# martinhoT/Footsies-Gym

Hardware: NVIDIA B200
Metric: env_frames_per_sec (higher is better)
Workload: dtype int32+fp32

## Files before the change

### footsies_gym_b200/csrc/footsies_kernels.cu

```cuda
#include <sched.h>
#include <stdlib.h>
#include <algorithm>

#include "rollout_kernel.h"
#include "step_kernel.cuh"

using namespace fg;
using namespace fgk;

namespace {

thread_local char g_err[512] = "";
int fail(int code, const char *fmt, const char *detail = "") {
    snprintf(g_err, sizeof g_err, fmt, detail);
    return code;
}
#define CUDA_TRY(expr) do { cudaError_t _e = (expr); if (_e != cudaSuccess) \
    return fail(FG_ERR_CUDA, #expr ": %s", cudaGetErrorString(_e)); } while (0)

}

struct fg_handle {
    fg_config cfg;
    fg_buffers buf;
    bool bound;
    Tables *d_tables;
    int sm_count;
    int64_t launches;
    int64_t step_calls;
    uint8_t *d_mask;
    int large_shape_min_envs;
    int pdl_min_envs;
    int host_chunk_envs;
    int host_lead_div;
    uint4 *d_packed;
    float *d_reward_table;
    uint32_t *d_pack_error;
    float h_reward_table[FG_PACKED_REWARD_TABLE_SIZE];
    int reward_table_count;
    float2 *d_position;
    uint8_t *d_obs_u8;
    cudaStream_t s_compute, s_copy;
    cudaEvent_t ev_fork, ev_join;
    std::vector<cudaEvent_t> ev_slice;
};

namespace {

int grid_for(const fg_handle *h, int blocks_per_sm) {
    int want = (h->cfg.num_envs + kThreads - 1) / kThreads;
    int cap = h->sm_count * blocks_per_sm;
    return want < cap ? (want > 0 ? want : 1) : cap;
}

Params make_params(const fg_handle *h, int first = 0, int count = -1) {
    Params p;
    memset(&p, 0, sizeof p);
    const size_t o = (size_t)first;
    p.pl_f1 = (uint4 *)h->buf.state[FG_PLANE_F1] + o; p.pl_f2 = (uint4 *)h->buf.state[FG_PLANE_F2] + o;
    p.pl_env = (uint4 *)h->buf.state[FG_PLANE_ENV] + o; p.pl_rng = (uint4 *)h->buf.state[FG_PLANE_RNG] + o;
    p.stats = (unsigned long long *)h->buf.stats;
    p.act1 = h->buf.actions_p1 ? h->buf.actions_p1 + o : nullptr;
    p.act2 = h->buf.actions_p2 ? h->buf.actions_p2 + o : nullptr;
    p.obs = (float4 *)h->buf.obs + 2 * o; p.reward = h->buf.reward + o; p.terminated = h->buf.terminated + o;
    p.info_frame = h->buf.info_frame + o; p.info_misc = (uint32_t *)h->buf.info_misc + o;
    p.step_mask = h->buf.step_mask ? h->buf.step_mask + o : nullptr;
    p.tables = h->d_tables;
    p.first_env_index = h->cfg.first_env_index + first;
    p.reverse = (int)(h->step_calls & 1);
    p.pdl = (count < 0 ? h->cfg.num_envs - first : count) >= h->pdl_min_envs;
    p.n = count < 0 ? h->cfg.num_envs - first : count; p.frame_skip = h->cfg.frame_skip; p.autoreset = h->cfg.autoreset;
    p.stale_intro = h->cfg.stale_intro_input;
    p.skip_unactionable = h->cfg.skip_unactionable;
    p.large_shape_min_envs = h->large_shape_min_envs;
    return p;
}

template <bool KF>
cudaError_t launch_step_k(const fg_config &c, int sm_count, cudaStream_t s, const Params &p) {
    const bool d = c.dense_reward != 0, m = p.step_mask != nullptr;
    if (c.p1_bot && c.p2_bot) return launch_step_d<KF, true, true>(d, m, sm_count, s, p);
    if (c.p1_bot) return launch_step_d<KF, true, false>(d, m, sm_count, s, p);
    if (c.p2_bot) return launch_step_d<KF, false, true>(d, m, sm_count, s, p);
    return launch_step_d<KF, false, false>(d, m, sm_count, s, p);
}

template <bool B1, bool B2>
cudaError_t launch_reset(int grid, cudaStream_t s, const Params &p) {
    static DeviceOnceFlags configured;
    if (cudaError_t e = configure_once_per_device(configured, [] {
            return cudaFuncSetAttribute(reset_kernel<B1, B2>, cudaFuncAttributeMaxDynamicSharedMemorySize, (int)sizeof(Tables)); }))
        return e;
    reset_kernel<B1, B2><<<grid, kThreads, sizeof(Tables), s>>>(p);
    return cudaSuccess;
}

int check_bound(const fg_handle *h) {
    if (!h) return fail(FG_ERR_INVALID_ARGUMENT, "null handle%s");
    if (!h->bound) return fail(FG_ERR_NOT_BOUND, "fg_bind has not been called%s");
    return FG_OK;
}

struct HostOut {
    float *obs_f32;
    float *position;
    uint8_t *obs_u8;
    float *reward;
    uint8_t *terminated;
    int32_t *info_frame;
    uint8_t *info_misc;
};

__global__ void __launch_bounds__(256) pack_obs_kernel(const float4 *__restrict__ obs, float2 *__restrict__ position,
                                                        uint8_t *__restrict__ obs_u8, int n) {
    const int pairs = n >> 1;
    for (int j = blockIdx.x * blockDim.x + threadIdx.x; j < pairs; j += gridDim.x * blockDim.x) {
        const float4 a0 = obs[4 * (size_t)j], a1 = obs[4 * (size_t)j + 1], b0 = obs[4 * (size_t)j + 2], b1 = obs[4 * (size_t)j + 3];
        reinterpret_cast<float4 *>(position)[j] = make_float4(a1.z, a1.w, b1.z, b1.w);
        const uint32_t A[6] = { (uint32_t)a0.x, (uint32_t)a0.y, (uint32_t)a0.z, (uint32_t)a0.w, (uint32_t)a1.x, (uint32_t)a1.y };
        const uint32_t B[6] = { (uint32_t)b0.x, (uint32_t)b0.y, (uint32_t)b0.z, (uint32_t)b0.w, (uint32_t)b1.x, (uint32_t)b1.y };
        uint32_t *o = reinterpret_cast<uint32_t *>(obs_u8) + 3 * (size_t)j;
        o[0] = A[0] | A[1] << 8 | A[2] << 16 | A[3] << 24;
        o[1] = A[4] | A[5] << 8 | B[0] << 16 | B[1] << 24;
        o[2] = B[2] | B[3] << 8 | B[4] << 16 | B[5] << 24;
    }
    if ((n & 1) && blockIdx.x == 0 && threadIdx.x == 0) {
        const int i = n - 1;
        const float4 a0 = obs[2 * (size_t)i], a1 = obs[2 * (size_t)i + 1];
        position[i] = make_float2(a1.z, a1.w);
        const float v[6] = { a0.x, a0.y, a0.z, a0.w, a1.x, a1.y };
        for (int k = 0; k < 6; k++) obs_u8[6 * (size_t)i + k] = (uint8_t)v[k];
    }
}

__global__ void __launch_bounds__(256) delay_ring_kernel(const float4 *__restrict__ obs, const int32_t *__restrict__ frame,
                                                         const uint32_t *__restrict__ misc, float4 *ring_obs, int32_t *ring_frame,
                                                         uint32_t *ring_misc, float4 *__restrict__ out_obs, int32_t *__restrict__ out_frame,
                                                         uint32_t *__restrict__ out_misc, const uint8_t *__restrict__ step_mask,
                                                         int n, int depth, int pos) {
    const int oldest = (pos + 1) % depth;
    for (int i = blockIdx.x * blockDim.x + threadIdx.x; i < n; i += gridDim.x * blockDim.x) {
        const int32_t f_now = frame[i];
        if ((step_mask && !step_mask[i]) || (f_now != -1 && f_now == ring_frame[(size_t)((pos + depth - 1) % depth) * n + i])) {
            const size_t last = (size_t)(depth - 1) * n + i;
            float4 ca = ring_obs[2 * last], cb = ring_obs[2 * last + 1];
            int32_t cf = ring_frame[last];
            uint32_t cm = ring_misc[last];
            for (int s = 0; s < depth; s++) {
                const size_t k = (size_t)s * n + i;
                const float4 ta = ring_obs[2 * k], tb = ring_obs[2 * k + 1];
                const int32_t tf = ring_frame[k];
                const uint32_t tm = ring_misc[k];
                ring_obs[2 * k] = ca; ring_obs[2 * k + 1] = cb; ring_frame[k] = cf; ring_misc[k] = cm;
                ca = ta; cb = tb; cf = tf; cm = tm;
            }
            continue;
        }
// ... 311 lines not shown
    if (cudaGetDeviceCount(&ndev) != cudaSuccess || device < 0 || device >= ndev) {
        cudaGetLastError();
        fail(FG_ERR_INVALID_ARGUMENT, "fg_host_alloc: no such device%s");
        return nullptr;
    }
    if (cudaSetDevice(device) != cudaSuccess) { fail(FG_ERR_CUDA, "fg_host_alloc: cudaSetDevice failed%s"); return nullptr; }
    cpu_set_t old_set, node_set;
    const int node = gpu_numa_node(device);
    const bool have_old = sched_getaffinity(0, sizeof old_set, &old_set) == 0;
    const bool bound = node >= 0 && have_old && node_cpuset(node, &node_set) && sched_setaffinity(0, sizeof node_set, &node_set) == 0;
    void *p = nullptr;
    cudaError_t e = cudaHostAlloc(&p, bytes ? bytes : 1, cudaHostAllocDefault);
    if (e == cudaSuccess) memset(p, 0, bytes);
    if (bound) sched_setaffinity(0, sizeof old_set, &old_set);
    if (e != cudaSuccess) { cudaGetLastError(); fail(FG_ERR_CUDA, "fg_host_alloc: cudaHostAlloc failed%s"); return nullptr; }
    return p;
}
void fg_host_free(void *p) { if (p) cudaFreeHost(p); }

int32_t fg_packed_reward_table(fg_handle *h, float *table, int32_t *count) {
    if (!h || !table || !count) return fail(FG_ERR_INVALID_ARGUMENT, "null argument%s");
    CUDA_TRY(cudaSetDevice(h->cfg.device));
    if (int rc = packed_init(h)) return rc;
    memcpy(table, h->h_reward_table, sizeof h->h_reward_table);
    *count = h->reward_table_count;
    return FG_OK;
}
int32_t fg_step_host_packed(fg_handle *h, const uint8_t *a1, const uint8_t *a2, fg_packed_result *out, void *stream) {
    return host_step_packed(h, a1, a2, out, (cudaStream_t)stream);
}
int32_t fg_reset_host_packed(fg_handle *h, const uint8_t *mask, fg_packed_result *out, void *stream) {
    return host_reset_packed(h, mask, out, (cudaStream_t)stream);
}

int32_t fg_abi_version(void) { return FG_ABI_VERSION; }
const char *fg_last_error(void) { return g_err; }

int32_t fg_algorithmic_bytes_per_env_step(const fg_config *cfg) {
    if (!cfg) return 0;
    const bool rng = cfg->p1_bot || cfg->p2_bot;
    int state = 2 * 16 * (rng ? 4 : 3);
    int actions = (cfg->p1_bot ? 0 : 1) + (cfg->p2_bot ? 0 : 1);
    return state + actions + 32  + 4  + 1  + 4  + 4 ;
}

int32_t fg_create(const fg_config *cfg, fg_handle **out) {
    if (!cfg || !out) return fail(FG_ERR_INVALID_ARGUMENT, "null argument%s");
    if (cfg->struct_size != (int32_t)sizeof(fg_config)) return fail(FG_ERR_INVALID_ARGUMENT, "fg_config.struct_size mismatch%s");
    if (cfg->num_envs <= 0) return fail(FG_ERR_INVALID_ARGUMENT, "num_envs must be positive%s");
    if (cfg->frame_skip < 1 || cfg->frame_skip > 64) return fail(FG_ERR_INVALID_ARGUMENT, "frame_skip must be in [1, 64]%s");
    if (cfg->skip_unactionable && cfg->p1_bot) return fail(FG_ERR_INVALID_ARGUMENT, "skip_unactionable needs an agent-controlled P1%s");
    int ndev = 0;
    if (cudaGetDeviceCount(&ndev) != cudaSuccess || ndev == 0) {
        cudaGetLastError();
        return fail(FG_ERR_NO_DEVICE, "no CUDA device: this library has no CPU fallback%s");
    }
    if (cfg->device < 0 || cfg->device >= ndev) return fail(FG_ERR_INVALID_ARGUMENT, "device ordinal out of range%s");
    CUDA_TRY(cudaSetDevice(cfg->device));
    fg_handle *h = new (std::nothrow) fg_handle();
    if (!h) return fail(FG_ERR_INVALID_STATE, "out of host memory%s");
    h->cfg = *cfg;
    h->bound = false;
    h->launches = 0;
    h->step_calls = 0;
    h->d_mask = nullptr;
    h->d_position = nullptr; h->d_obs_u8 = nullptr;
    h->d_packed = nullptr; h->d_reward_table = nullptr; h->d_pack_error = nullptr; h->reward_table_count = 0;
    h->s_compute = h->s_copy = nullptr;
    h->ev_fork = h->ev_join = nullptr;
    h->host_chunk_envs = 1024 * 1024;
    h->host_lead_div = 2;
    if (const char *v = getenv("FOOTSIES_B200_HOST_LEAD_DIV")) { const int d = atoi(v); if (d == 1 || d == 2 || d == 4) h->host_lead_div = d; }
    if (const char *v = getenv("FOOTSIES_B200_HOST_CHUNK_ENVS")) {
        const long long c = atoll(v);
        if (c >= 256) h->host_chunk_envs = (int)((c > (1ll << 30) ? (1ll << 30) : c) / 256 * 256);
    }
    h->large_shape_min_envs = kLargeShapeMinEnvs;
    if (const char *v = getenv("FOOTSIES_B200_LARGE_SHAPE_MIN_ENVS")) h->large_shape_min_envs = atoi(v);
    h->pdl_min_envs = (cfg->frame_skip > 1 || cfg->skip_unactionable) ? 262144 : 0;
    if (const char *v = getenv("FOOTSIES_B200_PDL_MIN_ENVS")) h->pdl_min_envs = atoi(v);
    cudaDeviceProp prop;
    CUDA_TRY(cudaGetDeviceProperties(&prop, cfg->device));
    h->sm_count = prop.multiProcessorCount;
    Tables *host = new Tables();
    build_tables(*host);
    cudaError_t e = cudaMalloc(&h->d_tables, sizeof(Tables));
    if (e == cudaSuccess) e = cudaMemcpy(h->d_tables, host, sizeof(Tables), cudaMemcpyHostToDevice);
    delete host;
    if (e != cudaSuccess) { delete h; return fail(FG_ERR_CUDA, "table upload: %s", cudaGetErrorString(e)); }
    *out = h;
    return FG_OK;
}

void fg_destroy(fg_handle *h) {
    if (!h) return;
    cudaSetDevice(h->cfg.device);
    cudaFree(h->d_tables);
    if (h->d_mask) cudaFree(h->d_mask);
    if (h->d_position) cudaFree(h->d_position);
    if (h->d_packed) { cudaFree(h->d_packed); cudaFree(h->d_reward_table); cudaFree(h->d_pack_error); }
    if (h->d_obs_u8) cudaFree(h->d_obs_u8);
    if (h->s_compute) { cudaStreamDestroy(h->s_compute); cudaStreamDestroy(h->s_copy); cudaEventDestroy(h->ev_fork); cudaEventDestroy(h->ev_join); }
    for (cudaEvent_t e : h->ev_slice) cudaEventDestroy(e);
    delete h;
}

int32_t fg_bind(fg_handle *h, const fg_buffers *b) {
    if (!h || !b) return fail(FG_ERR_INVALID_ARGUMENT, "null argument%s");
    if (b->struct_size != (int32_t)sizeof(fg_buffers)) return fail(FG_ERR_INVALID_ARGUMENT, "fg_buffers.struct_size mismatch%s");
    for (int k = 0; k < FG_STATE_PLANES; k++)
        if (!b->state[k] || ((uintptr_t)b->state[k] & 15u)) return fail(FG_ERR_INVALID_ARGUMENT, "state planes must be non-null and 16-byte aligned%s");
    if (!b->stats || !b->obs || !b->reward || !b->terminated || !b->info_frame || !b->info_misc)
        return fail(FG_ERR_INVALID_ARGUMENT, "output buffers must be non-null%s");
    if (((uintptr_t)b->obs & 15u) || ((uintptr_t)b->info_misc & 3u) || ((uintptr_t)b->stats & 7u))
        return fail(FG_ERR_INVALID_ARGUMENT, "obs must be 16-byte, info_misc 4-byte, stats 8-byte aligned%s");
    if (!h->cfg.p1_bot && !b->actions_p1) return fail(FG_ERR_INVALID_ARGUMENT, "actions_p1 is required unless p1_bot%s");
    if (!h->cfg.p2_bot && !b->actions_p2) return fail(FG_ERR_INVALID_ARGUMENT, "actions_p2 is required unless p2_bot%s");
    h->buf = *b;
    h->bound = true;
    return FG_OK;
}

int32_t fg_seed(fg_handle *h, int64_t seed_base, const uint8_t *mask, void *stream) {
    if (int rc = check_bound(h)) return rc;
    CUDA_TRY(cudaSetDevice(h->cfg.device));
    Params p = make_params(h);
    p.mask = mask; p.seed_base = seed_base;
    seed_kernel<<<grid_for(h, 8), kThreads, 0, (cudaStream_t)stream>>>(p);
    h->launches++;
    CUDA_TRY(cudaGetLastError());
    return FG_OK;
}

int32_t fg_reset(fg_handle *h, const uint8_t *mask, void *stream) {
    if (int rc = check_bound(h)) return rc;
    CUDA_TRY(cudaSetDevice(h->cfg.device));
    return reset_on(h, mask, (cudaStream_t)stream);
}

int32_t fg_step(fg_handle *h, void *stream) {
    if (int rc = check_bound(h)) return rc;
    CUDA_TRY(cudaSetDevice(h->cfg.device));
    h->step_calls++;
    return step_range(h, 0, -1, (cudaStream_t)stream);
}

int32_t fg_step_host(fg_handle *h, const uint8_t *a1, const uint8_t *a2, float *obs, float *reward,
                     uint8_t *terminated, int32_t *info_frame, uint8_t *info_misc, void *stream) {
    HostOut o = { obs, nullptr, nullptr, reward, terminated, info_frame, info_misc };
    return host_step(h, a1, a2, o, (cudaStream_t)stream);
}

int32_t fg_step_host_compact(fg_handle *h, const uint8_t *a1, const uint8_t *a2, const fg_host_outputs *out, void *stream) {
    if (!out || out->struct_size != (int32_t)sizeof(fg_host_outputs))
        return fail(FG_ERR_INVALID_ARGUMENT, "fg_host_outputs is null or its struct_size does not match%s");
    HostOut o = { nullptr, out->position, out->obs_u8, out->reward, out->terminated, out->info_frame, out->info_misc };
    return host_step(h, a1, a2, o, (cudaStream_t)stream);
}

int32_t fg_reset_host(fg_handle *h, const uint8_t *mask, float *obs, int32_t *info_frame, uint8_t *info_misc, void *stream) {
    HostOut o = { obs, nullptr, nullptr, nullptr, nullptr, info_frame, info_misc };
    return host_reset(h, mask, o, (cudaStream_t)stream);
}

int32_t fg_reset_host_compact(fg_handle *h, const uint8_t *mask, const fg_host_outputs *out, void *stream) {
    if (!out || out->struct_size != (int32_t)sizeof(fg_host_outputs))
// ... 154 lines not shown
```

### footsies_gym_b200/csrc/frame_logic.cuh

```cuda
#ifndef FOOTSIES_B200_FRAME_LOGIC_CUH
#define FOOTSIES_B200_FRAME_LOGIC_CUH

#include <stdint.h>

#include "state_codec.h"

#if defined(__CUDACC__)
#define FG_DEV __device__ __forceinline__
#define FG_ALIGN16 __align__(16)
namespace fg {
FG_DEV float u2f(uint32_t u) { return __uint_as_float(u); }
FG_DEV uint32_t f2u(float f) { return __float_as_uint(f); }
FG_DEV uint32_t umulhi64(uint32_t r, unsigned long long m) { return (uint32_t)__umul64hi((unsigned long long)r, m); }
FG_DEV uint32_t byte_lut(uint32_t lo, uint32_t hi, uint32_t idx) { return __byte_perm(lo, hi, idx); }
FG_DEV uint32_t umin(uint32_t a, uint32_t b) { return min(a, b); }
}
#else
#include <math.h>
#include <string.h>
#define FG_DEV static inline
#define FG_ALIGN16 alignas(16)
struct uint2 { uint32_t x, y; };
struct FG_ALIGN16 uint4 { uint32_t x, y, z, w; };
namespace fg {
// ... 214 lines not shown
    t2 = t2 < 4.0f ? 4.0f : t2 > 9.0f ? 9.0f : t2;
    return (uint32_t)((int)ceilf(t2) - 4);
}
FG_DEV float bot_dist_of_index(uint32_t idx) { return 0.5f * (float)(idx + 4u); }

template <int SIDE>
FG_DEV uint32_t bot_next(const Tables &T, Env &e, uint32_t &q, float dist, uint32_t opp_act) {
    uint32_t input = 0u;
    const bool have_m = (q & (127u << 9)) != 0u, have_a = (q & (127u << 24)) != 0u;
    if (have_m) {
        input = T.move_pat[SIDE][q & 511u];
        q += 1u - (1u << 9);
    }
    if (have_a) {
        input |= T.att_pat[(q >> 16) & 255u];
        q += (1u << 16) - (1u << 24);
    }
    if (!(have_m && have_a)) {
        const BotRow &b = T.bot[T.bucket_of[bot_dist_index(dist)]];
        if (!have_m) {
            const uint32_t r = rng_next(e);
            const uint32_t k = r - umulhi64(r, b.magic_m) * b.n_m;
            const uint32_t meta = T.move_meta[(b.sel_m >> (4u * k)) & 15u];
            q = (q & 0xffff0000u) | (meta & 0xffffu) | (meta >> 16) << 9;
        }
        if (!have_a) {
            const bool opp_hurt = opp_act == DAMAGE || opp_act == GUARD_BREAK || opp_act == N_SPECIAL || opp_act == B_SPECIAL;
            const bool opp_normal = opp_act == N_ATTACK || opp_act == B_ATTACK;
            uint32_t ap = 3u;
            if (!(opp_hurt || (opp_normal && (b.n_a >> 8)))) {
                const uint32_t r = rng_next(e);
                const uint32_t n = b.n_a & 255u;
                const uint32_t k = r - umulhi64(r, b.magic_a) * n;
                ap = (b.sel_a >> (4u * k)) & 15u;
            }
            const uint32_t meta = T.att_meta[ap];
            q = (q & 0x0000ffffu) | (meta & 0xffffu) << 16 | (meta >> 16) << 24;
        }
    }
    return input;
}

template <bool P1BOT, bool P2BOT>
FG_DEV void reset_env(const Tables &T, Env &e, bool stale_intro) {
    const bool was_done = (e.misc >> FGM_DONE_SHIFT) & 1u;
    uint32_t a1 = (e.misc >> FGM_ACTOR1_SHIFT) & 7u, a2 = (e.misc >> FGM_ACTOR2_SHIFT) & 7u;
    if (!stale_intro) { a1 = 0u; a2 = 0u; }
    float p1_dist = 0.0f;
    uint32_t p1_opp = 0u;
    bool p1_called = false;
    if (P1BOT) {
        p1_called = (e.misc >> FGM_P1CALLED_SHIFT) & 1u;
        p1_dist = was_done ? bot_dist_of_index((e.misc >> FGM_P1MEM_SHIFT) & 7u) : fabsf(e.pos2 - e.pos1);
        p1_opp = was_done ? (e.misc >> (FGM_P1MEM_SHIFT + 3)) & 31u : (e.pk2 >> FGP_ACT_SHIFT) & 31u;
    }
    uint32_t pk[2] = { e.pk1, e.pk2 };
    uint32_t npk[2];
#pragma unroll
    for (int s = 0; s < 2; s++) {
        uint32_t stun = (pk[s] >> FGP_STUN_SHIFT) & 31u;
        uint32_t keep = pk[s] & (M_INBACK | M_RPROX);
        if (was_done) {
            if (stun > 0u) stun--;
            if (!(pk[s] & M_VITAL)) keep = 0u;
        }
        uint32_t frame = 1u;
        if (stun > 0u) { stun--; frame = 0u; }
        npk[s] = STAND << FGP_ACT_SHIFT | frame << FGP_FRAME_SHIFT | stun << FGP_STUN_SHIFT | 3u << FGP_GUARD_SHIFT
               | M_VITAL | keep | FGP_CARRY_ALWAYS;
    }
    e.pk1 = npk[0]; e.pk2 = npk[1];
    e.pos1 = -2.0f; e.pos2 = 2.0f; e.vel1 = 0.0f; e.vel2 = 0.0f;
    e.hist1 = (T.dash_fsm[0][a1 & 3u] & 255u) | ((a1 >> 2) & 1u) << FGH_ARUN_SHIFT;
    e.hist2 = (T.dash_fsm[0][a2 & 3u] & 255u) | ((a2 >> 2) & 1u) << FGH_ARUN_SHIFT;
    e.frame = -1;
    e.bq2 = 0u;
    if (!P1BOT) e.bq1 = 0u;
    if (P1BOT) a1 = p1_called ? bot_next<0>(T, e, e.bq1, p1_dist, p1_opp) : 0u;
    if (P2BOT) a2 = bot_next<1>(T, e, e.bq2, 4.0f, STAND);
    e.misc = a1 << FGM_ACTOR1_SHIFT | a2 << FGM_ACTOR2_SHIFT
           | (P1BOT ? 1u << FGM_P1CALLED_SHIFT : 0u);
}

struct StepOutputs {
    float obs[8];
    uint32_t info_misc;
};
FG_DEV void make_outputs(const Env &e, StepOutputs &o) {
    uint32_t m1 = (e.pk1 >> FGP_ACT_SHIFT) & 31u, m2 = (e.pk2 >> FGP_ACT_SHIFT) & 31u;
    if (m1 >= DEAD) m1 = STAND;
    if (m2 >= DEAD) m2 = STAND;
    const uint32_t f1 = m1 <= BACKWARD ? 0u : e.pk1 & 63u;
    const uint32_t f2 = m2 <= BACKWARD ? 0u : e.pk2 & 63u;
    o.obs[0] = (float)((e.pk1 >> FGP_GUARD_SHIFT) & 3u); o.obs[1] = (float)((e.pk2 >> FGP_GUARD_SHIFT) & 3u);
    o.obs[2] = (float)m1; o.obs[3] = (float)m2;
    o.obs[4] = (float)f1; o.obs[5] = (float)f2; o.obs[6] = e.pos1; o.obs[7] = e.pos2;
    o.info_misc = ((e.misc >> FGM_REC1_SHIFT) & 7u) | ((e.misc >> FGM_REC2_SHIFT) & 7u) << 8
                | ((e.pk1 >> FGP_STUN_SHIFT) & 31u) << 16 | ((e.pk2 >> FGP_STUN_SHIFT) & 31u) << 24;
}

FG_DEV bool obs_is_skippable(const Env &e) {
    uint32_t m1 = (e.pk1 >> FGP_ACT_SHIFT) & 31u, m2 = (e.pk2 >> FGP_ACT_SHIFT) & 31u;
    if (m1 >= DEAD) m1 = STAND;
    if (m2 >= DEAD) m2 = STAND;
    const uint32_t f1 = m1 <= BACKWARD ? 0u : e.pk1 & 63u;
    const bool p2_hit_guard = m2 == DAMAGE || m2 == FT_IDX_GUARD_STAND || m2 == FT_IDX_GUARD_CROUCH || m2 == FT_IDX_GUARD_M || m2 == GUARD_BREAK;
    return (f1 != 0u && !p2_hit_guard) || m1 == DAMAGE;
}

template <bool P1BOT, bool P2BOT, bool DENSE, bool LUT_REQUEST>
FG_DEV void simulate_frame(const Tables &T, Env &e, uint32_t in1, uint32_t in2, double &reward, bool &terminal, StatAcc &acc) {
    float pre_dist = 0.0f;
    uint32_t pre_a1 = 0u, pre_a2 = 0u;
    if (P1BOT || P2BOT) {
        pre_dist = fabsf(e.pos2 - e.pos1);
        pre_a1 = (e.pk1 >> FGP_ACT_SHIFT) & 31u;
        pre_a2 = (e.pk2 >> FGP_ACT_SHIFT) & 31u;
    }

    e.frame++;
    if (e.frame < FG_MAX_RECORDING_INPUT_FRAME)
        e.misc = (e.misc & ~(63u << FGM_REC1_SHIFT)) | (in1 + in2 * 8u) << FGM_REC1_SHIFT;

    FrameOut f1, f2;
    update_fighter<0, LUT_REQUEST>(T, in1, e.pos1, e.vel1, e.pk1, e.hist1, f1);
    update_fighter<1, LUT_REQUEST>(T, in2, e.pos2, e.vel2, e.pk2, e.hist2, f2);

    const BoxCfg &b1 = boxcfg_of(T, f1.z), &b2 = boxcfg_of(T, f2.z);
    const float px1 = e.pos1 + u2f(b1.pcx), w1 = u2f(b1.pw);
    const float px2 = e.pos2 - u2f(b2.pcx), w2 = u2f(b2.pw);
    const float xmax1 = w1 + px1, xmax2 = w2 + px2;
    float s1 = 0.0f, s2 = 0.0f;
    if (xmax2 > px1 && px2 < xmax1) {
        if (e.pos1 < e.pos2) { const float d = xmax1 - px2; s1 = -0.5f * d; s2 = 0.5f * d; }
        else if (e.pos1 > e.pos2) { const float d = xmax2 - px1; s1 = 0.5f * d; s2 = -0.5f * d; }
    }
    float t1 = 0.0f, t2 = 0.0f;
    {
        const float c = px1 + s1, hw = 0.5f * w1, mn = c - hw, mx = c + hw;
        if (mn < -5.0f) t1 = -5.0f - mn; else if (mx > 5.0f) t1 = 5.0f - mx;
    }
    {
        const float c = px2 + s2, hw = 0.5f * w2, mn = c - hw, mx = c + hw;
        if (mn < -5.0f) t2 = -5.0f - mn; else if (mx > 5.0f) t2 = 5.0f - mx;
    }
    e.pos1 = (e.pos1 + s1) + t1;
    e.pos2 = (e.pos2 + s2) + t2;

    uint32_t res_a = 0u, res_b = 0u;
    if ((f1.z | f2.z) & (FT_Z_PROX | FT_Z_REAL)) {
        const AttackRow &ar1 = attack_of(T, f1.w), &ar2 = attack_of(T, f2.w);
        bool real_a, prox_a, real_b, prox_b;
        attack_overlaps<0>(ar1, b2, f1, f2, s1, t1, s2, t2, real_a, prox_a);
        attack_overlaps<1>(ar2, b1, f2, f1, s2, t2, s1, t1, real_b, prox_b);
        res_a = attack_apply<0>(ar1.result, e.pk1, e.pk2, f1, f2, real_a, prox_a, acc);
        res_b = attack_apply<1>(ar2.result, e.pk2, e.pk1, f2, f1, real_b, prox_b, acc);
    }

    if (f1.special_started && res_b == 0u) acc.s += f1.from_neutral ? 0x101u : 1u;

    terminal = ((e.pk1 & e.pk2) & M_VITAL) == 0u;

    if (DENSE) {
        const uint32_t code = (res_b >> 2) | (res_a >> 2) << 1;
        if (code | (terminal ? 1u : 0u)) {
            const uint32_t cum = T.cum_next[(e.misc >> FGM_CUM_SHIFT) & 15u][code];
// ... 25 lines not shown
```

### footsies_gym_b200/csrc/step_kernel.cuh

```cuda
#ifndef FOOTSIES_B200_STEP_KERNEL_CUH
#define FOOTSIES_B200_STEP_KERNEL_CUH
#include "device_once.h"
#include <cuda_runtime.h>
#include <stdint.h>
#include <stdio.h>
#include <string.h>
#include <new>
#include <vector>

#include "tables_host.h"

namespace fgk {

using namespace fg;

template <int THREADS_, int GROUP_, int STAGES_, int MIN_BLOCKS_>
struct StepShape {
    static constexpr int kThreads = THREADS_, kGroupThreads = GROUP_, kGroups = THREADS_ / GROUP_, kStages = STAGES_,
                         kMinBlocks = MIN_BLOCKS_;
    static_assert(THREADS_ % GROUP_ == 0 && GROUP_ % 32 == 0, "groups are whole warps");
};
#if defined(FG_THREADS)
#ifndef FG_GROUP
#define FG_GROUP FG_THREADS
#endif
#ifndef FG_STAGES
#define FG_STAGES 2
#endif
#ifndef FG_BLOCKS_PER_SM
#define FG_BLOCKS_PER_SM 4
#endif
using ShapeSmall = StepShape<FG_THREADS, FG_GROUP, FG_STAGES, FG_BLOCKS_PER_SM>;
using ShapeLargeSingle = ShapeSmall;
using ShapeLargeFused = ShapeSmall;
#else
using ShapeSmall = StepShape<256, 256, 2, 3>;
using ShapeLargeSingle = StepShape<768, 256, 3, 1>;
using ShapeLargeFused = StepShape<1024, 256, 3, 1>;
#endif
constexpr int kLargeShapeMinEnvs = 768 * 1024;
#ifndef FG_SKIP_RNG_STORE
#define FG_SKIP_RNG_STORE 1
#endif
#ifndef FG_PDL
#define FG_PDL 1
#endif
#ifndef FG_REVERSE
#define FG_REVERSE 1
#endif
constexpr int kThreads = 256;
constexpr uint32_t kFull = 0xffffffffu;

struct Params {
    uint4 *pl_f1, *pl_f2, *pl_env, *pl_rng;
    unsigned long long *stats;
    const uint8_t *act1, *act2;
    float4 *obs;
    float *reward;
    uint8_t *terminated;
    int32_t *info_frame;
    uint32_t *info_misc;
    const Tables *tables;
    const uint8_t *mask;
    const uint8_t *step_mask;
    long long seed_base, first_env_index;
    int n, frame_skip, autoreset, stale_intro;
    int skip_unactionable;
    int large_shape_min_envs;
    int reverse;
    int pdl;
    int pdl_min_envs;
};

__device__ __forceinline__ void write_outputs(const Params &p, int i, const Env &e, float reward, bool terminated) {
    StepOutputs o;
    make_outputs(e, o);
    p.obs[2 * (size_t)i] = make_float4(o.obs[0], o.obs[1], o.obs[2], o.obs[3]);
    p.obs[2 * (size_t)i + 1] = make_float4(o.obs[4], o.obs[5], o.obs[6], o.obs[7]);
    p.reward[i] = reward;
    p.terminated[i] = terminated ? 1 : 0;
    p.info_frame[i] = e.frame;
    p.info_misc[i] = o.info_misc;
}

__device__ __forceinline__ void load_tables(Tables *dst, const Tables *src) {
    const uint4 *s = reinterpret_cast<const uint4 *>(src);
    uint4 *d = reinterpret_cast<uint4 *>(dst);
    for (int k = threadIdx.x; k < (int)(sizeof(Tables) / 16); k += blockDim.x) d[k] = s[k];
}

template <bool WITH_RNG>
__device__ __forceinline__ void load_env(const Params &p, int i, Env &e) {
    const uint4 a = p.pl_f1[i], b = p.pl_f2[i], c = p.pl_env[i];
    e.pos1 = u2f(a.x); e.vel1 = u2f(a.y); e.pk1 = a.z; e.hist1 = a.w;
    e.pos2 = u2f(b.x); e.vel2 = u2f(b.y); e.pk2 = b.z; e.hist2 = b.w;
    e.frame = (int32_t)c.x; e.misc = c.y; e.bq2 = c.z; e.bq1 = c.w;
    if (WITH_RNG) { const uint4 r = p.pl_rng[i]; e.r0 = r.x; e.r1 = r.y; e.r2 = r.z; e.r3 = r.w; }
    e.drew = false;
}
template <bool WITH_RNG>
__device__ __forceinline__ void store_env(const Params &p, int i, const Env &e) {
    p.pl_f1[i] = make_uint4(f2u(e.pos1), f2u(e.vel1), e.pk1, e.hist1);
    p.pl_f2[i] = make_uint4(f2u(e.pos2), f2u(e.vel2), e.pk2, e.hist2);
    p.pl_env[i] = make_uint4((uint32_t)e.frame, e.misc, e.bq2, e.bq1);
    if (WITH_RNG && (!FG_SKIP_RNG_STORE || e.drew)) p.pl_rng[i] = make_uint4(e.r0, e.r1, e.r2, e.r3);
}

__device__ __forceinline__ void flush_stats(StatAcc &acc, unsigned long long *s_stats, int lane) {
    const uint32_t w[3] = { acc.a, acc.r, acc.s };
    const int map[3][4] = { { FG_STAT_EPISODES, FG_STAT_P1_WINS, FG_STAT_P2_WINS, FG_STAT_DOUBLE_KO },
                            { -1, FG_STAT_HITS, FG_STAT_BLOCKS, FG_STAT_GUARD_BREAKS },
                                            { FG_STAT_P1_SPECIALS, FG_STAT_P1_SPECIALS_NEUTRAL, FG_STAT_RESETS, FG_STAT_ENV_FRAMES } };
#pragma unroll
    for (int k = 0; k < 3; k++)
#pragma unroll
        for (int b = 0; b < 4; b++) {
            if (map[k][b] < 0) continue;
            const uint32_t tot = __reduce_add_sync(kFull, (w[k] >> (8 * b)) & 255u);
            if (lane == 0 && tot) atomicAdd(&s_stats[map[k][b]], (unsigned long long)tot);
        }
    const uint32_t lo = __reduce_add_sync(kFull, acc.ep_frames & 0xffffu), hi = __reduce_add_sync(kFull, acc.ep_frames >> 16);
    if (lane == 0 && (lo | hi)) atomicAdd(&s_stats[FG_STAT_EPISODE_FRAMES], ((unsigned long long)hi << 16) + lo);
    acc.a = 0u; acc.r = 0u; acc.s = 0u; acc.ep_frames = 0u;
}

__device__ __forceinline__ uint32_t smem_u32(const void *p) { return (uint32_t)__cvta_generic_to_shared(p); }
__device__ __forceinline__ void mbar_init(uint64_t *bar, uint32_t count) {
    asm volatile("mbarrier.init.shared::cta.b64 [%0], %1;" ::"r"(smem_u32(bar)), "r"(count));
}
__device__ __forceinline__ void mbar_expect_tx(uint64_t *bar, uint32_t bytes) {
    asm volatile("mbarrier.arrive.expect_tx.shared::cta.b64 _, [%0], %1;" ::"r"(smem_u32(bar)), "r"(bytes) : "memory");
}
__device__ __forceinline__ void mbar_arrive(uint64_t *bar) {
    asm volatile("mbarrier.arrive.shared::cta.b64 _, [%0];" ::"r"(smem_u32(bar)) : "memory");
}
__device__ __forceinline__ void mbar_wait(uint64_t *bar, uint32_t parity) {
    asm volatile(
        "{\n"
        ".reg .pred P1;\n"
        "LAB_WAIT:\n"
        "mbarrier.try_wait.parity.shared::cta.b64 P1, [%0], %1;\n"
        "@P1 bra DONE;\n"
        "bra LAB_WAIT;\n"
        "DONE:\n"
        "}" ::"r"(smem_u32(bar)), "r"(parity) : "memory");
}
__device__ __forceinline__ void tma_load_1d(void *dst, const void *src, uint32_t bytes, uint64_t *bar) {
    asm volatile("cp.async.bulk.shared::cluster.global.mbarrier::complete_tx::bytes [%0], [%1], %2, [%3];"
                 ::"r"(smem_u32(dst)), "l"(src), "r"(bytes), "r"(smem_u32(bar)) : "memory");
}

template <class SH, int PLANES>
struct __align__(128) StepSmem {
    Tables T;
    uint4 stage[SH::kGroups][SH::kStages][PLANES][SH::kGroupThreads];
    uint64_t full_bar[SH::kGroups][SH::kStages], empty_bar[SH::kGroups][SH::kStages];
    unsigned long long stats[FG_STAT_COUNT];
};

template <class SH, bool KFUSED, bool P1BOT, bool P2BOT, bool DENSE, bool MASKED>
__global__ void __launch_bounds__(SH::kThreads, SH::kMinBlocks) step_kernel(const Params p) {
    constexpr bool kRng = P1BOT || P2BOT;
    constexpr int kPlanes = kRng ? 4 : 3;
    constexpr int kGroupThreads = SH::kGroupThreads, kGroups = SH::kGroups, kStages = SH::kStages;
    extern __shared__ __align__(128) unsigned char smem_raw[];
    StepSmem<SH, kPlanes> &S = *reinterpret_cast<StepSmem<SH, kPlanes> *>(smem_raw);
    const Tables &T = S.T;
    const int lane = threadIdx.x & 31;
    const int g = threadIdx.x / kGroupThreads, lt = threadIdx.x % kGroupThreads;
    const int num_chunks = (p.n + kGroupThreads - 1) / kGroupThreads;
    const int full_chunks = p.n / kGroupThreads;
    const int first = blockIdx.x * kGroups + g, stride = gridDim.x * kGroups;
    const uint4 *const planes[4] = { p.pl_f1, p.pl_f2, p.pl_env, p.pl_rng };
    auto issue = [&](int chunk, int s) {
        mbar_expect_tx(&S.full_bar[g][s], (uint32_t)(kPlanes * kGroupThreads * sizeof(uint4)));
#pragma unroll
        for (int k = 0; k < kPlanes; k++)
            tma_load_1d(S.stage[g][s][k], planes[k] + (size_t)chunk * kGroupThreads, (uint32_t)(kGroupThreads * sizeof(uint4)),
                        &S.full_bar[g][s]);
    };
    auto chunk_of = [&](int c) { return (FG_REVERSE && p.reverse && c < full_chunks) ? full_chunks - 1 - c : c; };
    if (lt == 0) {
        for (int s = 0; s < kStages; s++) { mbar_init(&S.full_bar[g][s], 1u); mbar_init(&S.empty_bar[g][s], kGroupThreads / 32); }
        asm volatile("fence.mbarrier_init.release.cluster;" ::: "memory");
    }
    if (FG_PDL && p.pdl) {
        load_tables(&S.T, p.tables);
        if (threadIdx.x < FG_STAT_COUNT) S.stats[threadIdx.x] = 0ull;
        asm volatile("griddepcontrol.launch_dependents;" ::: "memory");
        asm volatile("griddepcontrol.wait;" ::: "memory");
    }
    if (lt == 0) {
        for (int j = 0; j < kStages - 1; j++) {
            const int cj = first + j * stride;
            if (cj < num_chunks && chunk_of(cj) < full_chunks) issue(chunk_of(cj), j);
        }
    }
    if (!(FG_PDL && p.pdl)) {
        load_tables(&S.T, p.tables);
        if (threadIdx.x < FG_STAT_COUNT) S.stats[threadIdx.x] = 0ull;
    }
    __syncthreads();
    StatAcc acc = { 0u, 0u, 0u, 0u };
    uint32_t frames_since_flush = 0u;
    uint32_t nin1 = 0u, nin2 = 0u;
    {
        const int i0 = (first < num_chunks ? chunk_of(first) : num_chunks) * kGroupThreads + lt;
        if (i0 < p.n) { if (!P1BOT) nin1 = p.act1[i0]; if (!P2BOT) nin2 = p.act2[i0]; }
    }
    int k = 0;
    for (int cl = first; cl < num_chunks; cl += stride, k++) {
        const int s = k % kStages;
        const int c = chunk_of(cl);
        const int i = c * kGroupThreads + lt;
        const bool staged = c < full_chunks;
        bool valid = staged || i < p.n;
        if (MASKED) valid = valid && p.step_mask[valid ? i : 0] != 0;
        if (lt == 0) {
            const int cn = cl + (kStages - 1) * stride;
            if (cn < num_chunks && chunk_of(cn) < full_chunks) {
                const int sn = (k + kStages - 1) % kStages;
                if (k >= 1) mbar_wait(&S.empty_bar[g][sn], ((k - 1) / kStages) & 1);
                issue(chunk_of(cn), sn);
            }
        }
        const uint32_t act1 = nin1, act2 = nin2;
        {
            const int cn1 = cl + stride;
            const int in = (cn1 < num_chunks ? chunk_of(cn1) : num_chunks) * kGroupThreads + lt;
            if (in < p.n) { if (!P1BOT) nin1 = p.act1[in]; if (!P2BOT) nin2 = p.act2[in]; }
        }
        Env e;
        bool run = false;
        uint32_t in1 = 0u, in2 = 0u;
        if (staged) {
            mbar_wait(&S.full_bar[g][s], (k / kStages) & 1);
            const uint4 a = S.stage[g][s][0][lt], b = S.stage[g][s][1][lt], cc = S.stage[g][s][2][lt];
            e.pos1 = u2f(a.x); e.vel1 = u2f(a.y); e.pk1 = a.z; e.hist1 = a.w;
            e.pos2 = u2f(b.x); e.vel2 = u2f(b.y); e.pk2 = b.z; e.hist2 = b.w;
            e.frame = (int32_t)cc.x; e.misc = cc.y; e.bq2 = cc.z; e.bq1 = cc.w;
            if (kRng) { const uint4 r = S.stage[g][s][kPlanes - 1][lt]; e.r0 = r.x; e.r1 = r.y; e.r2 = r.z; e.r3 = r.w; }
            e.drew = false;
            __syncwarp();
            if (lane == 0) mbar_arrive(&S.empty_bar[g][s]);
        } else if (valid) {
            load_env<kRng>(p, i, e);
        }
        if (valid) {
            if ((e.misc >> FGM_DONE_SHIFT) & 1u) {
                if (p.autoreset) {
                    reset_env<P1BOT, P2BOT>(T, e, p.stale_intro != 0);
                    store_env<kRng>(p, i, e);
                    write_outputs(p, i, e, 0.0f, false);
                    acc.s += 0x10000u;
                } else {
                    p.reward[i] = 0.0f;
                }
            } else {
                run = true;
                in1 = P1BOT ? (e.misc >> FGM_ACTOR1_SHIFT) & 7u : act1 & 7u;
                in2 = P2BOT ? (e.misc >> FGM_ACTOR2_SHIFT) & 7u : act2 & 7u;
            }
        }
        double reward = 0.0;
        bool terminal = false;
        const int K = KFUSED ? p.frame_skip : 1;
        for (int kk = 0; kk < K; kk++) {
            if (run && !terminal) {
                simulate_frame<P1BOT, P2BOT, DENSE, KFUSED>(T, e, in1, in2, reward, terminal, acc);
                acc.s += 1u << 24;
                if (KFUSED) {
                    if (P1BOT) in1 = (e.misc >> FGM_ACTOR1_SHIFT) & 7u;
                    if (P2BOT) in2 = (e.misc >> FGM_ACTOR2_SHIFT) & 7u;
                }
            }
        }
        if (KFUSED && p.skip_unactionable) {
            bool more = run && !terminal && obs_is_skippable(e);
            while (__any_sync(kFull, more)) {
                for (int kk = 0; kk < K; kk++) {
                    if (more && !terminal) {
                        simulate_frame<P1BOT, P2BOT, DENSE, KFUSED>(T, e, 0u, in2, reward, terminal, acc);
                        acc.s += 1u << 24;
                        if (P2BOT) in2 = (e.misc >> FGM_ACTOR2_SHIFT) & 7u;
                    }
                }
                more = more && !terminal && obs_is_skippable(e);
                frames_since_flush += (uint32_t)K;
                if (frames_since_flush >= kStatFlushFrames) { flush_stats(acc, S.stats, lane); frames_since_flush = 0u; }
            }
        }
        if (run) {
            store_env<kRng>(p, i, e);
            write_outputs(p, i, e, (float)reward, terminal);
        }
        frames_since_flush += (uint32_t)K;
        if (frames_since_flush >= kStatFlushFrames) { flush_stats(acc, S.stats, lane); frames_since_flush = 0u; }
    }
    flush_stats(acc, S.stats, lane);
    __syncthreads();
    if (threadIdx.x < FG_STAT_COUNT && S.stats[threadIdx.x]) atomicAdd(&p.stats[threadIdx.x], S.stats[threadIdx.x]);
}

template <bool P1BOT, bool P2BOT>
__global__ void __launch_bounds__(kThreads) reset_kernel(const Params p) {
    extern __shared__ __align__(128) unsigned char smem_raw[];
    Tables &T = *reinterpret_cast<Tables *>(smem_raw);
    load_tables(&T, p.tables);
    __syncthreads();
    constexpr bool kRng = P1BOT || P2BOT;
    unsigned long long resets = 0ull;
    for (int i = blockIdx.x * blockDim.x + threadIdx.x; i < p.n; i += gridDim.x * blockDim.x) {
        if (p.mask && !p.mask[i]) continue;
        Env e;
        load_env<kRng>(p, i, e);
        reset_env<P1BOT, P2BOT>(T, e, p.stale_intro != 0);
        store_env<kRng>(p, i, e);
        write_outputs(p, i, e, 0.0f, false);
        resets++;
    }
    if (resets) atomicAdd(&p.stats[FG_STAT_RESETS], resets);
}

static __global__ void __launch_bounds__(kThreads) seed_kernel(const Params p) {
    for (int i = blockIdx.x * blockDim.x + threadIdx.x; i < p.n; i += gridDim.x * blockDim.x) {
        if (p.mask && !p.mask[i]) continue;
        uint32_t s0 = (uint32_t)(int32_t)(p.seed_base + p.first_env_index + i);
        uint32_t s1 = s0 * 1812433253u + 1u, s2 = s1 * 1812433253u + 1u, s3 = s2 * 1812433253u + 1u;
        p.pl_rng[i] = make_uint4(s0, s1, s2, s3);
    }
}

template <class SH, bool KF, bool B1, bool B2, bool D, bool M>
cudaError_t launch_step_shape(int sm_count, cudaStream_t s, const Params &p) {
    constexpr int kPlanes = (B1 || B2) ? 4 : 3;
    constexpr size_t bytes = sizeof(StepSmem<SH, kPlanes>);
    static DeviceOnceFlags configured;
    if (cudaError_t e = configure_once_per_device(configured, [] {
            return cudaFuncSetAttribute(step_kernel<SH, KF, B1, B2, D, M>, cudaFuncAttributeMaxDynamicSharedMemorySize, (int)bytes); }))
        return e;
    const int want = (p.n + SH::kThreads - 1) / SH::kThreads, cap = sm_count * SH::kMinBlocks;
    const int grid = want < cap ? (want > 0 ? want : 1) : cap;
#if FG_PDL
    if (!p.pdl) {
        step_kernel<SH, KF, B1, B2, D, M><<<grid, SH::kThreads, bytes, s>>>(p);
        return cudaSuccess;
    }
    cudaLaunchConfig_t cfg = {};
    cfg.gridDim = dim3((unsigned)grid);
    cfg.blockDim = dim3((unsigned)SH::kThreads);
    cfg.dynamicSmemBytes = bytes;
    cfg.stream = s;
    cudaLaunchAttribute attr[1];
    attr[0].id = cudaLaunchAttributeProgrammaticStreamSerialization;
    attr[0].val.programmaticStreamSerializationAllowed = 1;
    cfg.attrs = attr;
    cfg.numAttrs = 1;
    return cudaLaunchKernelEx(&cfg, step_kernel<SH, KF, B1, B2, D, M>, p);
#else
    step_kernel<SH, KF, B1, B2, D, M><<<grid, SH::kThreads, bytes, s>>>(p);
    return cudaSuccess;
#endif
}
template <bool KF, bool B1, bool B2, bool D, bool M>
cudaError_t launch_step(int sm_count, cudaStream_t s, const Params &p) {
    if (p.n < p.large_shape_min_envs) return launch_step_shape<ShapeSmall, KF, B1, B2, D, M>(sm_count, s, p);
    if (KF) return launch_step_shape<ShapeLargeFused, KF, B1, B2, D, M>(sm_count, s, p);
    return launch_step_shape<ShapeLargeSingle, KF, B1, B2, D, M>(sm_count, s, p);
}
template <bool KF, bool B1, bool B2>
cudaError_t launch_step_d(bool dense, bool masked, int sm_count, cudaStream_t s, const Params &p) {
    if (dense) return masked ? launch_step<KF, B1, B2, true, true>(sm_count, s, p) : launch_step<KF, B1, B2, true, false>(sm_count, s, p);
    return masked ? launch_step<KF, B1, B2, false, true>(sm_count, s, p) : launch_step<KF, B1, B2, false, false>(sm_count, s, p);
}
#ifndef FG_STEP_INSTANCE
extern template cudaError_t launch_step_d<false, false, false>(bool, bool, int, cudaStream_t, const Params &);
extern template cudaError_t launch_step_d<false, false, true>(bool, bool, int, cudaStream_t, const Params &);
extern template cudaError_t launch_step_d<false, true, false>(bool, bool, int, cudaStream_t, const Params &);
extern template cudaError_t launch_step_d<false, true, true>(bool, bool, int, cudaStream_t, const Params &);
extern template cudaError_t launch_step_d<true, false, false>(bool, bool, int, cudaStream_t, const Params &);
extern template cudaError_t launch_step_d<true, false, true>(bool, bool, int, cudaStream_t, const Params &);
extern template cudaError_t launch_step_d<true, true, false>(bool, bool, int, cudaStream_t, const Params &);
extern template cudaError_t launch_step_d<true, true, true>(bool, bool, int, cudaStream_t, const Params &);
#endif

}
#endif
```

Baseline: 34.18 billion.

## Add streaming cache hints and on-demand RNG loads for large step launches

When the env count exceeds what fits in L2, the large single-frame shape now uses streaming (evict-first) stores for outputs and streaming loads for actions, so per-step traffic does not evict state. In the non-fused bot path the RNG plane is no longer staged through shared memory; it is loaded from global only when a bot may draw, which shrinks the staging footprint and skips reads. An optional evict-last store for state and a stage-count macro are added but disabled by default. The trade-offs are scattered uncoalesced RNG loads on the compute path, and the L2-size threshold heuristic may mis-set when hints turn on.

```diff
diff --git a/footsies_gym_b200/csrc/footsies_kernels.cu b/footsies_gym_b200/csrc/footsies_kernels.cu
--- a/footsies_gym_b200/csrc/footsies_kernels.cu
+++ b/footsies_gym_b200/csrc/footsies_kernels.cu
@@ -31,6 +31,7 @@
     uint8_t *d_mask;
     int large_shape_min_envs;
     int pdl_min_envs;
+    long long cache_hint_min_envs;
     int host_chunk_envs;
     int host_lead_div;
     uint4 *d_packed;
@@ -73,6 +74,7 @@
     p.stale_intro = h->cfg.stale_intro_input;
     p.skip_unactionable = h->cfg.skip_unactionable;
     p.large_shape_min_envs = h->large_shape_min_envs;
+    p.cache_hints = p.n >= h->cache_hint_min_envs;
     return p;
 }
 
@@ -550,6 +552,11 @@
     cudaDeviceProp prop;
     CUDA_TRY(cudaGetDeviceProperties(&prop, cfg->device));
     h->sm_count = prop.multiProcessorCount;
+    int l2_bytes = 0;
+    CUDA_TRY(cudaDeviceGetAttribute(&l2_bytes, cudaDevAttrL2CacheSize, cfg->device));
+    const long long footprint = FG_STATE_PLANES * 16 + 32  + 4  + 1  + 4  + 4 ;
+    h->cache_hint_min_envs = (long long)l2_bytes / footprint + 1;
+    if (const char *v = getenv("FOOTSIES_B200_CACHE_HINT_MIN_ENVS")) h->cache_hint_min_envs = atoll(v);
     Tables *host = new Tables();
     build_tables(*host);
     cudaError_t e = cudaMalloc(&h->d_tables, sizeof(Tables));
diff --git a/footsies_gym_b200/csrc/frame_logic.cuh b/footsies_gym_b200/csrc/frame_logic.cuh
--- a/footsies_gym_b200/csrc/frame_logic.cuh
+++ b/footsies_gym_b200/csrc/frame_logic.cuh
@@ -320,6 +320,14 @@
            | (P1BOT ? 1u << FGM_P1CALLED_SHIFT : 0u);
 }
 
+template <bool P1BOT, bool P2BOT>
+FG_DEV bool bot_may_draw(const Env &e) {
+    bool may = ((e.misc >> FGM_DONE_SHIFT) & 1u) != 0u;
+    if (P2BOT) may = may || (e.bq2 & (127u << 9)) == 0u || (e.bq2 & (127u << 24)) == 0u;
+    if (P1BOT) may = may || (e.bq1 & (127u << 9)) == 0u || (e.bq1 & (127u << 24)) == 0u;
+    return may;
+}
+
 struct StepOutputs {
     float obs[8];
     uint32_t info_misc;
diff --git a/footsies_gym_b200/csrc/step_kernel.cuh b/footsies_gym_b200/csrc/step_kernel.cuh
--- a/footsies_gym_b200/csrc/step_kernel.cuh
+++ b/footsies_gym_b200/csrc/step_kernel.cuh
@@ -6,6 +6,7 @@
 #include <stdio.h>
 #include <string.h>
 #include <new>
+#include <type_traits>
 #include <vector>
 
 #include "tables_host.h"
@@ -20,6 +21,9 @@
                          kMinBlocks = MIN_BLOCKS_;
     static_assert(THREADS_ % GROUP_ == 0 && GROUP_ % 32 == 0, "groups are whole warps");
 };
+#ifndef FG_LARGE_STAGES
+#define FG_LARGE_STAGES 3
+#endif
 #if defined(FG_THREADS)
 #ifndef FG_GROUP
 #define FG_GROUP FG_THREADS
@@ -35,7 +39,7 @@
 using ShapeLargeFused = ShapeSmall;
 #else
 using ShapeSmall = StepShape<256, 256, 2, 3>;
-using ShapeLargeSingle = StepShape<768, 256, 3, 1>;
+using ShapeLargeSingle = StepShape<768, 256, FG_LARGE_STAGES, 1>;
 using ShapeLargeFused = StepShape<1024, 256, 3, 1>;
 #endif
 constexpr int kLargeShapeMinEnvs = 768 * 1024;
@@ -47,6 +51,15 @@
 #endif
 #ifndef FG_REVERSE
 #define FG_REVERSE 1
+#endif
+#ifndef FG_RNG_ON_DEMAND
+#define FG_RNG_ON_DEMAND 1
+#endif
+#ifndef FG_CACHE_HINTS
+#define FG_CACHE_HINTS 1
+#endif
+#ifndef FG_EVICT_LAST_STATE
+#define FG_EVICT_LAST_STATE 0
 #endif
 constexpr int kThreads = 256;
 constexpr uint32_t kFull = 0xffffffffu;
@@ -70,17 +83,29 @@
     int reverse;
     int pdl;
     int pdl_min_envs;
+    int cache_hints;
 };
 
-__device__ __forceinline__ void write_outputs(const Params &p, int i, const Env &e, float reward, bool terminated) {
+template <bool KFUSED, bool P1BOT, bool P2BOT>
+struct StepPlanes { static constexpr int value = (P1BOT || P2BOT) && (KFUSED || !FG_RNG_ON_DEMAND) ? 4 : 3; };
+
+template <class T>
+__device__ __forceinline__ void st_out(T *ptr, T v, bool evict_first) {
+    if (evict_first) __stcs(ptr, v); else *ptr = v;
+}
+template <class T>
+__device__ __forceinline__ T ld_act(const T *ptr, bool evict_first) { return evict_first ? __ldcs(ptr) : *ptr; }
+
+__device__ __forceinline__ void write_outputs(const Params &p, int i, const Env &e, float reward, bool terminated,
+                                              bool evict_first = false) {
     StepOutputs o;
     make_outputs(e, o);
-    p.obs[2 * (size_t)i] = make_float4(o.obs[0], o.obs[1], o.obs[2], o.obs[3]);
-    p.obs[2 * (size_t)i + 1] = make_float4(o.obs[4], o.obs[5], o.obs[6], o.obs[7]);
-    p.reward[i] = reward;
-    p.terminated[i] = terminated ? 1 : 0;
-    p.info_frame[i] = e.frame;
-    p.info_misc[i] = o.info_misc;
+    st_out(&p.obs[2 * (size_t)i], make_float4(o.obs[0], o.obs[1], o.obs[2], o.obs[3]), evict_first);
+    st_out(&p.obs[2 * (size_t)i + 1], make_float4(o.obs[4], o.obs[5], o.obs[6], o.obs[7]), evict_first);
+    st_out(&p.reward[i], reward, evict_first);
+    st_out(&p.terminated[i], (uint8_t)(terminated ? 1 : 0), evict_first);
+    st_out(&p.info_frame[i], (int32_t)e.frame, evict_first);
+    st_out(&p.info_misc[i], o.info_misc, evict_first);
 }
 
 __device__ __forceinline__ void load_tables(Tables *dst, const Tables *src) {
@@ -98,11 +123,21 @@
     if (WITH_RNG) { const uint4 r = p.pl_rng[i]; e.r0 = r.x; e.r1 = r.y; e.r2 = r.z; e.r3 = r.w; }
     e.drew = false;
 }
+__device__ __forceinline__ void st_evict_last(uint4 *ptr, uint4 v) {
+    uint64_t pol;
+    asm("createpolicy.fractional.L2::evict_last.b64 %0, 1.0;" : "=l"(pol));
+    asm volatile("st.global.L2::cache_hint.v4.u32 [%0], {%1, %2, %3, %4}, %5;"
+                 ::"l"(ptr), "r"(v.x), "r"(v.y), "r"(v.z), "r"(v.w), "l"(pol) : "memory");
+}
 template <bool WITH_RNG>
-__device__ __forceinline__ void store_env(const Params &p, int i, const Env &e) {
-    p.pl_f1[i] = make_uint4(f2u(e.pos1), f2u(e.vel1), e.pk1, e.hist1);
-    p.pl_f2[i] = make_uint4(f2u(e.pos2), f2u(e.vel2), e.pk2, e.hist2);
-    p.pl_env[i] = make_uint4((uint32_t)e.frame, e.misc, e.bq2, e.bq1);
+__device__ __forceinline__ void store_env(const Params &p, int i, const Env &e, bool evict_last = false) {
+    const uint4 a = make_uint4(f2u(e.pos1), f2u(e.vel1), e.pk1, e.hist1), b = make_uint4(f2u(e.pos2), f2u(e.vel2), e.pk2, e.hist2),
+                c = make_uint4((uint32_t)e.frame, e.misc, e.bq2, e.bq1);
+    if (FG_EVICT_LAST_STATE && evict_last) {
+        st_evict_last(&p.pl_f1[i], a); st_evict_last(&p.pl_f2[i], b); st_evict_last(&p.pl_env[i], c);
+    } else {
+        p.pl_f1[i] = a; p.pl_f2[i] = b; p.pl_env[i] = c;
+    }
     if (WITH_RNG && (!FG_SKIP_RNG_STORE || e.drew)) p.pl_rng[i] = make_uint4(e.r0, e.r1, e.r2, e.r3);
 }
 
@@ -161,7 +196,10 @@
 template <class SH, bool KFUSED, bool P1BOT, bool P2BOT, bool DENSE, bool MASKED>
 __global__ void __launch_bounds__(SH::kThreads, SH::kMinBlocks) step_kernel(const Params p) {
     constexpr bool kRng = P1BOT || P2BOT;
-    constexpr int kPlanes = kRng ? 4 : 3;
+    constexpr int kPlanes = StepPlanes<KFUSED, P1BOT, P2BOT>::value;
+    constexpr bool kRngStaged = kRng && kPlanes == 4;
+    constexpr bool kHints = FG_CACHE_HINTS && !KFUSED && std::is_same<SH, ShapeLargeSingle>::value;
+    const bool hints = kHints && p.cache_hints;
     constexpr int kGroupThreads = SH::kGroupThreads, kGroups = SH::kGroups, kStages = SH::kStages;
     extern __shared__ __align__(128) unsigned char smem_raw[];
     StepSmem<SH, kPlanes> &S = *reinterpret_cast<StepSmem<SH, kPlanes> *>(smem_raw);
@@ -206,7 +244,7 @@
     uint32_t nin1 = 0u, nin2 = 0u;
     {
         const int i0 = (first < num_chunks ? chunk_of(first) : num_chunks) * kGroupThreads + lt;
-        if (i0 < p.n) { if (!P1BOT) nin1 = p.act1[i0]; if (!P2BOT) nin2 = p.act2[i0]; }
+        if (i0 < p.n) { if (!P1BOT) nin1 = ld_act(p.act1 + i0, hints); if (!P2BOT) nin2 = ld_act(p.act2 + i0, hints); }
     }
     int k = 0;
     for (int cl = first; cl < num_chunks; cl += stride, k++) {
@@ -214,6 +252,7 @@
         const int c = chunk_of(cl);
         const int i = c * kGroupThreads + lt;
         const bool staged = c < full_chunks;
+        const bool evict_last = kHints && FG_EVICT_LAST_STATE && hints && cl + FG_EVICT_LAST_STATE * stride >= num_chunks;
         bool valid = staged || i < p.n;
         if (MASKED) valid = valid && p.step_mask[valid ? i : 0] != 0;
         if (lt == 0) {
@@ -228,7 +267,7 @@
         {
             const int cn1 = cl + stride;
             const int in = (cn1 < num_chunks ? chunk_of(cn1) : num_chunks) * kGroupThreads + lt;
-            if (in < p.n) { if (!P1BOT) nin1 = p.act1[in]; if (!P2BOT) nin2 = p.act2[in]; }
+            if (in < p.n) { if (!P1BOT) nin1 = ld_act(p.act1 + in, hints); if (!P2BOT) nin2 = ld_act(p.act2 + in, hints); }
         }
         Env e;
         bool run = false;
@@ -239,10 +278,13 @@
             e.pos1 = u2f(a.x); e.vel1 = u2f(a.y); e.pk1 = a.z; e.hist1 = a.w;
             e.pos2 = u2f(b.x); e.vel2 = u2f(b.y); e.pk2 = b.z; e.hist2 = b.w;
             e.frame = (int32_t)cc.x; e.misc = cc.y; e.bq2 = cc.z; e.bq1 = cc.w;
-            if (kRng) { const uint4 r = S.stage[g][s][kPlanes - 1][lt]; e.r0 = r.x; e.r1 = r.y; e.r2 = r.z; e.r3 = r.w; }
+            if (kRngStaged) { const uint4 r = S.stage[g][s][kPlanes - 1][lt]; e.r0 = r.x; e.r1 = r.y; e.r2 = r.z; e.r3 = r.w; }
             e.drew = false;
             __syncwarp();
             if (lane == 0) mbar_arrive(&S.empty_bar[g][s]);
+            if (kRng && !kRngStaged && valid && bot_may_draw<P1BOT, P2BOT>(e)) {
+                const uint4 r = p.pl_rng[i]; e.r0 = r.x; e.r1 = r.y; e.r2 = r.z; e.r3 = r.w;
+            }
         } else if (valid) {
             load_env<kRng>(p, i, e);
         }
@@ -250,8 +292,8 @@
             if ((e.misc >> FGM_DONE_SHIFT) & 1u) {
                 if (p.autoreset) {
                     reset_env<P1BOT, P2BOT>(T, e, p.stale_intro != 0);
-                    store_env<kRng>(p, i, e);
-                    write_outputs(p, i, e, 0.0f, false);
+                    store_env<kRng>(p, i, e, evict_last);
+                    write_outputs(p, i, e, 0.0f, false, hints);
                     acc.s += 0x10000u;
                 } else {
                     p.reward[i] = 0.0f;
@@ -291,8 +333,8 @@
             }
         }
         if (run) {
-            store_env<kRng>(p, i, e);
-            write_outputs(p, i, e, (float)reward, terminal);
+            store_env<kRng>(p, i, e, evict_last);
+            write_outputs(p, i, e, (float)reward, terminal, hints);
         }
         frames_since_flush += (uint32_t)K;
         if (frames_since_flush >= kStatFlushFrames) { flush_stats(acc, S.stats, lane); frames_since_flush = 0u; }
@@ -333,7 +375,7 @@
 
 template <class SH, bool KF, bool B1, bool B2, bool D, bool M>
 cudaError_t launch_step_shape(int sm_count, cudaStream_t s, const Params &p) {
-    constexpr int kPlanes = (B1 || B2) ? 4 : 3;
+    constexpr int kPlanes = StepPlanes<KF, B1, B2>::value;
     constexpr size_t bytes = sizeof(StepSmem<SH, kPlanes>);
     static DeviceOnceFlags configured;
     if (cudaError_t e = configure_once_per_device(configured, [] {
```

Result: slower. 28.18 billion, median of 6 (-17.6%).
